# kleinzcy/speech_signal_processing

Hardware: AMD Instinct MI355X
Metric: MFCC frames/s (one fused pass: framing .. DCT + delta + delta-delta, 39-d) (higher is better)
Workload: dtype f32; 1 GPU; configs[1]: 100000 x 3 s synthetic 16 kHz utterances per GPU, 39-d MFCC (+delta+delta-delta), 400/160/512, 24 mel; utterances_per_gpu=100000, frames_per_gpu=29800000, d_out=39, parallelism=utterance-sharded x1, world_size_observed=1

## Files before the change

### speech_signal_processing_amd/csrc/mfcc.hpp

```cpp
#pragma once
#include "common.hpp"

namespace ssp {

struct MfccChunk {
    int32_t utt;
    int32_t t0;
    int32_t n;
    int32_t pad;
};

struct MfccArgs {
    const float* samples;
    const int64_t* sample_off;
    const int64_t* frame_off;
    float* out;
    float* lm_out;
    const MfccChunk* chunks;
    float* utt_max;
    const float* window;
    const float2* twiddle;
    const int32_t* filt_lo4;
    const float* filt_wT;
    const int32_t* filt_grp;
    int32_t filt_w4_total;
    int32_t dct_identity;
    int32_t dct_ncp;
    const float* dct;
    const float* dctT;
    int32_t win_len, hop, n_fft, n_filt, n_ceps, d_out;
    int32_t frame_mode, preemph_mode, spec_power, log_mode, floor_mode, delta_order, delta_N, cmvn;
    float preemph, spec_scale, eps, top_db, delta_inv_denom;
    int32_t lds_logmel_off, lds_ceps_off, lds_dlt_off, lds_ddl_off, lds_lmrows_off, lds_stats_off, lds_tw_off;
    int32_t lds_dct_off;
    int32_t lds_wt_off;
    int32_t lm_stride;
    int32_t n_chunks;
    int32_t prefetch;
};

constexpr int MFCC_FAST_MAX_PASS = 4;

struct FastArgs {
    const float2* tw16;
    const float2* wpost;
    const float* melw;
    const int32_t* mel_lo;
    const int32_t* mel_id;
    const float* dctT;
    int32_t mel_steps[MFCC_FAST_MAX_PASS];
    int32_t mel_blocks[MFCC_FAST_MAX_PASS];
    int32_t lm_pad;
    int32_t n_pass, q_pass, total_steps, n_filt4;
    float ddw[17];
    int32_t slen;
    int32_t stage_floats;
    int32_t ceps_rows;
    int32_t off_win, off_tw16, off_wpost, off_melw, off_mello, off_melid, off_dct, off_ceps, off_stats, off_wave, wave_bytes;
    float pscale;
    float one_minus_a;
    const float* pc_w;
    const int32_t* pc_ofs;
    const float* pc_mask;
    const int32_t* pc_fid;
    int32_t melv;
    int32_t mel_ns;
    float log_add, log_max, log_k;
    float* ceps_scratch;
    int32_t* work_counter;
    int32_t* redo_flags;
    int32_t ceps_stride;
    int32_t n_chunks;
};

struct StreamArgs {
    const float* dctA;
    int32_t* work_counter;
    int32_t* redo_flags;
    int32_t n_chunks;
    int32_t wave_bytes;
    int32_t stage_bytes;
    int32_t table_bytes;
    int32_t tstep;
    const float* dense_w;
};

int launch_mfcc_generic(const MfccArgs& args, int n_chunks, size_t lds_bytes, int n_waves, int num_cu, hipStream_t stream);
int launch_cmvn(const float* in, float* out, const int64_t* frame_off_dev, int64_t n_utt, int dim, int64_t max_T, hipStream_t stream);
int launch_topdb_dct(const float* logmel, const int64_t* frame_off_dev, int64_t n_utt, const MfccChunk* chunks, int n_chunks,
                     const float* utt_max, int n_filt, int n_ceps, const float* dct, float top_db, float* out, hipStream_t stream);
    

}

struct ssp_mfcc_plan {
    ssp_ctx* ctx = nullptr;
    ssp_mfcc_cfg cfg{};
    int32_t d_out = 0;
    bool reproducible = false;
    ssp::DevBuf window, twiddle, filt_lo4, filt_grp, filt_wT, dct, dctT, fbank_dense;
    int32_t max_filt_len = 0;
    uint64_t checked_sseg = 0, checked_fseg = 0;
    uint64_t cache_sseg = 0;
    uint64_t cache_fseg = 0;
    int cache_variant = -1;
    int cache_request = -1;
    bool cache_split_cmvn = false;
    bool cache_split_topdb = false;
    ssp::DevBuf lm_scratch, umax_scratch;
    int cache_chunk_frames = 0;
    size_t cache_lds = 0;
    int cache_waves = 4;
    int32_t cache_n_chunks = 0;
    std::vector<int32_t> cache_chunk_first;
    ssp::DevBuf chunks;
    ssp::MfccArgs args{};
    bool fast_ready = false;
    int64_t fast_max_samples = 0;
    ssp::FastArgs fast{};
    ssp::DevBuf f_tw16, f_wpost, f_melw, f_mello, f_melid, f_dct, f_pcw, f_pcofs, f_pcmask, f_pcfid, f_scratch, f_counter;
    bool stream_ready = false;
    ssp::DevBuf s_dctA, s_dense;
    bool cache_s2k_fused = false;
    bool s2k_ready = false;
    int32_t s2k_steps = 0, s2k_steps1 = 0;
    ssp::DevBuf s2k_twA, s2k_twB, s2k_twS, s2k_mel, s2k_minfo;
};

namespace ssp {
bool mfcc_fast_supported(const ssp_mfcc_cfg& cfg);
int build_fast_tables(ssp_mfcc_plan* plan);
size_t mfcc_fast_lds(const ssp_mfcc_cfg& cfg, FastArgs& f, int chunk_frames);
int mfcc_fast_max_chunk(const ssp_mfcc_cfg& cfg, const FastArgs& f);
int launch_mfcc_fast(const MfccArgs& args, ssp_mfcc_plan* plan, int n_chunks, int chunk_frames, hipStream_t stream);
bool mfcc_stream_supported(const ssp_mfcc_plan* plan);
bool mfcc_s2k_supported(const ssp_mfcc_plan* plan);
int build_s2k_tables(ssp_mfcc_plan* plan);
bool mfcc_s2k_fuses(const ssp_mfcc_plan* plan, int64_t max_T, int chunk_frames);
int launch_mfcc_s2k(const MfccArgs& args, ssp_mfcc_plan* plan, int n_chunks, hipStream_t stream);
bool mfcc_stream_dense(const ssp_mfcc_plan* plan);
bool mfcc_stream_fuses_cmvn(const ssp_mfcc_plan* plan);
int build_stream_tables(ssp_mfcc_plan* plan);
int launch_mfcc_stream(const MfccArgs& args, ssp_mfcc_plan* plan, int n_chunks, hipStream_t stream, bool dry_run = false);
}
```

### speech_signal_processing_amd/csrc/mfcc_plan.hip

```cpp
#include <chrono>
#include <cmath>
#include <cstdlib>

#include "mfcc.hpp"

namespace ssp {

static int validate_cfg(const ssp_mfcc_cfg* c) {
    if (!c) SSP_FAIL(SSP_ERR_INVALID, "mfcc: null cfg");
    if (c->n_fft < 64 || c->n_fft > 2048 || (c->n_fft & (c->n_fft - 1)))
        SSP_FAIL(SSP_ERR_UNSUPPORTED, "mfcc: n_fft=%d must be a power of two in [64, 2048]", c->n_fft);
    if (c->win_len < 1 || c->win_len > c->n_fft) SSP_FAIL(SSP_ERR_INVALID, "mfcc: win_len=%d not in [1, n_fft]", c->win_len);
    if (c->hop < 1) SSP_FAIL(SSP_ERR_INVALID, "mfcc: hop < 1");
    if (c->n_filt < 1 || c->n_filt > 512) SSP_FAIL(SSP_ERR_INVALID, "mfcc: n_filt=%d not in [1,512]", c->n_filt);
    if (c->n_ceps < 1 || c->n_ceps > 128) SSP_FAIL(SSP_ERR_INVALID, "mfcc: n_ceps=%d not in [1,128]", c->n_ceps);
    if (c->frame_mode < 0 || c->frame_mode > 2) SSP_FAIL(SSP_ERR_INVALID, "mfcc: frame_mode");
    if (c->frame_mode == 2 && c->win_len != c->n_fft)
        SSP_FAIL(SSP_ERR_UNSUPPORTED, "mfcc: centred framing needs win_len == n_fft");
    if (c->preemph_mode < 0 || c->preemph_mode > 1) SSP_FAIL(SSP_ERR_INVALID, "mfcc: preemph_mode");
    if (c->spec_power != 1 && c->spec_power != 2) SSP_FAIL(SSP_ERR_INVALID, "mfcc: spec_power must be 1 or 2");
    if (c->log_mode < 0 || c->log_mode > 2) SSP_FAIL(SSP_ERR_INVALID, "mfcc: log_mode");
    if (c->floor_mode < 0 || c->floor_mode > 2) SSP_FAIL(SSP_ERR_INVALID, "mfcc: floor_mode");
    if (c->delta_order < 0 || c->delta_order > 2) SSP_FAIL(SSP_ERR_INVALID, "mfcc: delta_order must be 0, 1 or 2");
    if (c->delta_order > 0 && (c->delta_N < 1 || c->delta_N > 8))
// ... 94 lines not shown
            MfccArgs probe = p->args;
            probe.cmvn = (c.cmvn != 0 && !split_cmvn) ? 1 : 0;
            const int prc = launch_mfcc_stream(probe, p, 0, nullptr, true);
            if (prc != SSP_OK) return prc;
        }
    } else if (variant == 2) {
        FastArgs tmp = p->fast;
        const int cap = mfcc_fast_max_chunk(c, tmp);
        ch = (int)std::min<int64_t>(std::max<int64_t>(max_T, 1), std::min(512, cap));
        if (whole) {
            ch = (int)std::max<int64_t>(max_T, 1);
            if (ch > cap) {
                split_cmvn = true;
                whole = false;
                ch = (int)std::min<int64_t>(std::max<int64_t>(max_T, 1), std::min(512, cap));
            }
        }
        lds = mfcc_fast_lds(c, tmp, ch);
        if (lds > lds_cap) SSP_FAIL(SSP_ERR_UNSUPPORTED, "mfcc(fast): LDS footprint %zu B exceeds 160 KiB", lds);
    } else {
        MfccArgs tmp = p->args;
        size_t half_cap = (size_t)(c.n_fft >= 2048 ? 80 : (c.n_fft >= 1024 ? 53 : 40)) * 1024;
        if (const char* e = getenv("SSP_GENERIC_LDS_CAP_KB")) half_cap = (size_t)atoi(e) * 1024;
        auto chunk_for = [&](const ssp_mfcc_cfg& cc) {
            int k = (int)std::min<int64_t>(std::max<int64_t>(max_T, 1), 512);
            while (k > 16 && generic_lds_layout(cc, k, 4, &tmp) > half_cap) k = (k * 3) / 4;
            return k;
        };
        nw = 4;
        ch = chunk_for(c);
        if (whole) {
            ch = (int)std::max<int64_t>(max_T, 1);
            if (generic_lds_layout(c, ch, 8, &tmp) <= lds_cap) {
                nw = 8;
            } else if (generic_lds_layout(c, ch, 4, &tmp) > lds_cap) {
                if (c.top_db >= 0.f) {
                    if (c.delta_order != 0 || c.cmvn)
                        SSP_FAIL(SSP_ERR_UNSUPPORTED,
                                 "mfcc: top_db with deltas / cmvn needs a whole utterance per workgroup; %lld frames exceed the 160 KiB LDS",
                                 (long long)max_T);
                    split_topdb = true;
                } else {
                    split_cmvn = true;
                }
                whole = false;
                ch = chunk_for(c);
                if (split_topdb) {
                    ssp_mfcc_cfg c2 = c;
                    c2.top_db = -1.f;
                    ch = chunk_for(c2);
                }
            }
        }
        {
            ssp_mfcc_cfg c2 = c;
            if (split_topdb) c2.top_db = -1.f;
            lds = generic_lds_layout(c2, ch, nw, &p->args);
        }
        if (lds > lds_cap) SSP_FAIL(SSP_ERR_UNSUPPORTED, "mfcc: LDS footprint %zu B exceeds 160 KiB", lds);
    }
    std::vector<MfccChunk> chunks;
    chunks.reserve((size_t)fseg->n);
    int64_t tail_from = fseg->n;
#ifndef SSP_NO_TAIL_SPLIT
    if (variant == 3 && !(c.cmvn != 0 && !split_cmvn) && !getenv("SSP_MFCC_NO_TAIL_SPLIT")) {
        const int64_t waves = (int64_t)p->ctx->num_cu * 12;
        if (fseg->n >= 4 * waves) tail_from = fseg->n - waves;
    }
#endif
    p->cache_chunk_first.assign((size_t)fseg->n + 1, 0);
    for (int64_t u = 0; u < fseg->n; ++u) {
        const int64_t T = fseg->host[u + 1] - fseg->host[u];
        if (T > INT32_MAX) SSP_FAIL(SSP_ERR_UNSUPPORTED, "mfcc: utterance %lld has too many frames", (long long)u);
        p->cache_chunk_first[(size_t)u] = (int32_t)std::min<size_t>(chunks.size(), (size_t)INT32_MAX);
        int64_t chu = ch;
        if (u >= tail_from && T >= 64) chu = std::min<int64_t>(ch, ((T + 1) / 2 + 15) / 16 * 16);
        const int pad = (variant == 3 && (!small_batch || repro)) ? 12 : 0;
        for (int64_t t0 = 0; t0 < T; t0 += chu)
            chunks.push_back(MfccChunk{(int32_t)u, (int32_t)t0, (int32_t)std::min<int64_t>(chu, T - t0), t0 > 0 ? pad : 0});
    }
    if (chunks.size() > (size_t)INT32_MAX) SSP_FAIL(SSP_ERR_UNSUPPORTED, "mfcc: too many chunks");
    p->cache_chunk_first[(size_t)fseg->n] = (int32_t)chunks.size();
    SSP_TRY(upload(p->chunks, chunks, p->ctx->stream));
    SSP_HIP(hipStreamSynchronize(p->ctx->stream));
    p->fast_max_samples = sseg->max_len();
    p->cache_n_chunks = (int32_t)chunks.size();
    p->cache_chunk_frames = ch;
    p->cache_lds = lds;
    p->cache_waves = nw;
    p->cache_sseg = sseg->serial;
    p->cache_fseg = fseg->serial;
    p->cache_variant = variant;
    p->cache_split_cmvn = split_cmvn;
    p->cache_split_topdb = split_topdb;
    return SSP_OK;
}

}

using namespace ssp;

extern "C" {

int ssp_mfcc_num_frames(const ssp_mfcc_cfg* cfg, int64_t n_samples, int64_t* n_frames) {
    if (!cfg || !n_frames || n_samples < 0) SSP_FAIL(SSP_ERR_INVALID, "ssp_mfcc_num_frames: bad argument");
    if (cfg->hop < 1 || cfg->frame_mode < 0 || cfg->frame_mode > 2) SSP_FAIL(SSP_ERR_INVALID, "ssp_mfcc_num_frames: bad cfg");
    *n_frames = frames_for(*cfg, n_samples);
    return SSP_OK;
}

int ssp_mfcc_out_dim(const ssp_mfcc_cfg* cfg, int32_t* d_out) {
    if (!cfg || !d_out) SSP_FAIL(SSP_ERR_INVALID, "ssp_mfcc_out_dim: null");
    *d_out = cfg->n_ceps * (1 + cfg->delta_order);
    return SSP_OK;
}

int ssp_mfcc_plan_create(ssp_ctx* ctx, const ssp_mfcc_cfg* cfg, const float* window, const float* fbank,
                         const float* dct, ssp_mfcc_plan** out) {
    ssp::TraceRange trace_("ssp_mfcc_plan_create");
    if (!out) SSP_FAIL(SSP_ERR_INVALID, "ssp_mfcc_plan_create: null out");
    *out = nullptr;
    SSP_TRY(use_ctx(ctx));
    SSP_TRY(validate_cfg(cfg));
    if (!window || !fbank || !dct) SSP_FAIL(SSP_ERR_INVALID, "ssp_mfcc_plan_create: null table");
    ssp_mfcc_plan* p = new (std::nothrow) ssp_mfcc_plan;
    if (!p) SSP_FAIL(SSP_ERR_NOMEM, "mfcc plan: host alloc");
    p->ctx = ctx;
    p->cfg = *cfg;
    p->d_out = cfg->n_ceps * (1 + cfg->delta_order);
    const int n_fft = cfg->n_fft, nb = n_fft / 2 + 1;

    std::vector<float> win(n_fft, 0.f);
    for (int i = 0; i < cfg->win_len; ++i) win[i] = window[i];
    std::vector<float2> tw(n_fft);
    for (int k = 0; k < n_fft; ++k) {
        const double ang = -2.0 * M_PI * (double)k / (double)n_fft;
        tw[k] = make_float2((float)cos(ang), (float)sin(ang));
    }
    std::vector<int32_t> lo(cfg->n_filt), len(cfg->n_filt), ofs(cfg->n_filt);
    std::vector<float> w;
    int32_t maxlen = 0;
    for (int j = 0; j < cfg->n_filt; ++j) {
        const float* row = fbank + (size_t)j * nb;
        int first = -1, last = -1;
        for (int k = 0; k < nb; ++k)
            if (row[k] != 0.f) {
                if (first < 0) first = k;
                last = k;
            }
        lo[j] = first < 0 ? 0 : first;
        len[j] = first < 0 ? 0 : last - first + 1;
        ofs[j] = (int32_t)w.size();
        for (int k = 0; k < len[j]; ++k) w.push_back(row[lo[j] + k]);
        maxlen = std::max(maxlen, len[j]);
    }
    p->max_filt_len = maxlen;
    const int n_grp = (cfg->n_filt + 63) / 64;
    std::vector<int32_t> lo4(cfg->n_filt);
    std::vector<float> wT;
    MfccArgs& ga = p->args;
    const int buf_floats = n_fft + n_fft / 16;
    std::vector<int32_t> grp(16, 0);
    for (int g = 0; g < n_grp; ++g) {
        const int j1 = std::min(cfg->n_filt, g * 64 + 64);
        int32_t steps = 2, taps = 0;
        for (int pass = 0; pass < 8; ++pass) {
// ... 493 lines not shown
```

### speech_signal_processing_amd/csrc/mfcc_stream_kernel.hpp

```cpp
#pragma once
#include <algorithm>
#include <cmath>
#include <cstdlib>
#include <type_traits>

#include "mfcc.hpp"
#include "cplx.hpp"

namespace ssp {

namespace {
typedef unsigned v2u __attribute__((ext_vector_type(2)));
typedef __attribute__((address_space(3))) const volatile v2f* lds_cv2f_t;
typedef __attribute__((address_space(3))) const volatile float* lds_cvf_t;
constexpr int ZROW = 128;
constexpr int ZFRAME = 16 * ZROW;
constexpr int LM_OFF = 1792;
constexpr int RING_FRAMES = 24;
constexpr int RING_ROW = 64;
constexpr int STREAM_WAVES = 4;
#ifndef SSP_S_PSHIFT
#define SSP_S_PSHIFT 64
#endif
constexpr int PSH = SSP_S_PSHIFT;
static_assert(4 * (256 + 24) + PSH <= LM_OFF - 192, "shifted P row: piece reads must stay below the log-mel rows");
#define SSP_STR_(x) #x
#define SSP_STR(x) SSP_STR_(x)

__device__ __forceinline__ float stream_log(const FastArgs& f, float v) {
    return __builtin_amdgcn_logf(fmaxf(v + f.log_add, f.log_max)) * f.log_k;
}

__device__ __forceinline__ float delta_weight(float t, float tp, float Tm1, float half_inv) {
    const float lo = tp <= 0.f ? -1.0e6f : tp;
    const float hi = tp >= Tm1 ? 1.0e6f : tp;
    const float a = fmaxf(lo, t - 2.f), b = fminf(hi, t + 2.f);
    const float cnt = fmaxf(b - a + 1.f, 0.f);
    const float w = cnt * (a + b - 2.f * t) * half_inv;
    return (tp < 0.f || tp > Tm1) ? 0.f : w;
}
}

template <int NZ, int POWER, int PRE, int MELV, int KS, int NS, int OCC, int CM, int WALK>
__global__ __launch_bounds__(64 * STREAM_WAVES, OCC) void mfcc_stream512_kernel(MfccArgs a, FastArgs f, StreamArgs sa) {
    extern __shared__ __attribute__((aligned(16))) char smem[];
    if (WALK && sa.work_counter[1] == 0) return;
    const int tid = threadIdx.x, lane = tid & 63;
    const int wave = __builtin_amdgcn_readfirstlane(tid >> 6);
    const int g = lane >> 4, j = lane & 15;
    constexpr int nc = 13;
    constexpr int mel_ns = NS;

    char* zbuf = smem + wave * sa.wave_bytes;
    float* stage = reinterpret_cast<float*>(zbuf + 4 * ZFRAME);
    char* ring = zbuf + 4 * ZFRAME + sa.stage_bytes;

    v2f wreg[NZ];
#pragma unroll
    for (int n1 = 0; n1 < NZ; ++n1) wreg[n1] = *reinterpret_cast<const v2f*>(a.window + 32 * n1 + 2 * j);
#pragma unroll
    for (int n1 = 0; n1 < NZ; ++n1) wreg[n1] = edge_row_taps(wreg[n1], 32 * n1 + 2 * j, a.win_len);
#ifndef SSP_STREAM_NTW
#define SSP_STREAM_NTW 15
#endif
#ifndef SSP_STREAM_NTW_CM
#define SSP_STREAM_NTW_CM 12
#endif
#ifndef SSP_STREAM_NWP
#define SSP_STREAM_NWP 8
#endif
    constexpr int NTW = OCC >= 3 ? (CM ? SSP_STREAM_NTW_CM : ((MELV <= 3 && NS <= 2) ? SSP_STREAM_NTW : ((MELV >= 4 && NS >= 4) ? 8 : 9))) : 15, NWP = OCC >= 3 ? SSP_STREAM_NWP : 8;
    static_assert(NTW >= 8, "rows above NTW take W^((k1 - 8) j) W^(8 j): W^(8 j) = twr[7] must be resident");
    v2f twr[NTW], wpr[NWP];
#pragma unroll
    for (int k1 = 1; k1 <= NTW; ++k1) twr[k1 - 1] = *reinterpret_cast<const v2f*>(&f.tw16[k1 * 16 + j]);
    float dA[KS];
#pragma unroll
    for (int s = 0; s < KS; ++s) dA[s] = sa.dctA[s * 64 + lane];
#pragma unroll
    for (int i = 0; i < NWP; ++i) wpr[i] = *reinterpret_cast<const v2f*>(&f.wpost[i * 16 + j]);
    constexpr bool DENSE = MELV == 0;
    constexpr int MV = DENSE ? 1 : MELV;
    v4f mw[MV];
    int mofs[MV];
    v2f mk01 = v2f{0.f, 0.f}, mk23 = v2f{0.f, 0.f};
    int mfid = -1;
    v4f dw[DENSE ? 6 : 1][4];
    float dw256[DENSE ? 6 : 1];
    if (DENSE) {
#pragma unroll
        for (int k = 0; k < 6; ++k) {
#pragma unroll
            for (int i = 0; i < 4; ++i) dw[DENSE ? k : 0][i] = *reinterpret_cast<const v4f*>(sa.dense_w + ((size_t)lane * 6 + k) * 20 + 4 * i);
            dw256[DENSE ? k : 0] = sa.dense_w[((size_t)lane * 6 + k) * 20 + 16];
        }
    } else {
#pragma unroll
        for (int i = 0; i < MV; ++i) {
            mw[i] = *reinterpret_cast<const v4f*>(f.pc_w + ((size_t)lane * MV + i) * 4);
            mofs[i] = f.pc_ofs[lane * MV + i];
        }
        mk01 = *reinterpret_cast<const v2f*>(f.pc_mask + lane * 4);
        mk23 = NS > 2 ? *reinterpret_cast<const v2f*>(f.pc_mask + lane * 4 + 2) : v2f{0.f, 0.f};
        mfid = f.pc_fid[lane];
    }

    const int hop = a.hop;
    const float pre = PRE ? a.preemph : 0.f;
    const float npre = -pre;
    const int n_piece = (f.slen + 255) >> 8;
    const bool has_half = (f.slen & 255) != 0 && (f.slen & 255) <= 128;
    const int n_full = has_half ? n_piece - 1 : n_piece;
    const int dord = a.delta_order;
    const int Dd = a.d_out;
    const float half_inv = 0.5f * a.delta_inv_denom;
    const uint32_t stage_lds = __builtin_amdgcn_readfirstlane((uint32_t)(uintptr_t)(lds_ptr_t)stage);

#ifdef SSP_S_CLOCK
    const unsigned long long ck0 = __builtin_amdgcn_s_memtime(), rt0 = __builtin_amdgcn_s_memrealtime();
#endif
    uint64_t wm = 0;
    int wblk = blockIdx.x * STREAM_WAVES + wave, wbase = 0;
    for (;;) {
        int cidx = 0;
        if constexpr (WALK) {
            bool done = false;
            while (wm == 0) {
                if ((int64_t)wblk * 64 >= sa.n_chunks) {
                    done = true;
                    break;
                }
                const int idx = wblk * 64 + lane;
                const int fl = idx < sa.n_chunks ? sa.redo_flags[idx] : 0;
                wm = __builtin_amdgcn_ballot_w64(fl != 0);
                wbase = wblk * 64;
                wblk += gridDim.x * STREAM_WAVES;
            }
            if (done) break;
            cidx = __builtin_amdgcn_readfirstlane(wbase + __builtin_ctzll(wm));
            wm &= wm - 1;
        } else {
            if (lane == 0) cidx = atomicAdd(sa.work_counter, 1);
            cidx = __builtin_amdgcn_readfirstlane(cidx);
            if (cidx >= sa.n_chunks) break;
        }
        const MfccChunk ch = a.chunks[cidx];
        const int64_t s0 = a.sample_off[ch.utt];
        const int64_t N = a.sample_off[ch.utt + 1] - s0;
        const int64_t f0 = a.frame_off[ch.utt];
        const int T = __builtin_amdgcn_readfirstlane((int)(a.frame_off[ch.utt + 1] - f0));
        const int t0 = __builtin_amdgcn_readfirstlane(ch.t0), n = __builtin_amdgcn_readfirstlane(ch.n);
        const int H = dord > 0 ? 4 : 0;
        const int Hlo = dord > 0 ? H + __builtin_amdgcn_readfirstlane(ch.pad) : 0;
        const int ta = max(t0 - Hlo, 0), tb = min(t0 + n + H, T);
        const int R = tb - ta;
        const int nquads = (R + 3) >> 2;
        const int E = t0 + n - ta;
        const int n_steps = (E + 4 + 15) >> 4;
        const int Q = DENSE ? nquads : 4 * n_steps;
        const float Tm1 = (float)(T - 1);

        const uint64_t xaddr = reinterpret_cast<uint64_t>(a.samples + s0);
        const uint32_t xlo = __builtin_amdgcn_readfirstlane((uint32_t)xaddr), xhi = __builtin_amdgcn_readfirstlane((uint32_t)(xaddr >> 32));
        const int xbytes = __builtin_amdgcn_readfirstlane((int)(N * 4));
        const __amdgpu_buffer_rsrc_t rs = __builtin_amdgcn_make_buffer_rsrc(
            reinterpret_cast<float*>(((uint64_t)xhi << 32) | xlo), 0, xbytes, 0x00020000);
        const uint64_t oaddr = reinterpret_cast<uint64_t>(a.out + (size_t)f0 * Dd);
        const uint32_t olo = __builtin_amdgcn_readfirstlane((uint32_t)oaddr), ohi = __builtin_amdgcn_readfirstlane((uint32_t)(oaddr >> 32));
        const __amdgpu_buffer_rsrc_t ro = __builtin_amdgcn_make_buffer_rsrc(
            reinterpret_cast<float*>(((uint64_t)ohi << 32) | olo), 0, __builtin_amdgcn_readfirstlane(T * Dd * 4), 0x00020000);

        auto prefetch = [&](int q) {
            const int vo = (ta + 4 * q) * hop * 4 + lane * 16;
            const lds_ptr_t lp = (lds_ptr_t)(uintptr_t)stage_lds;
            if (n_full > 0) __builtin_amdgcn_raw_ptr_buffer_load_lds(rs, lp, 16, vo, 0, 0, 0);
            if (n_full > 1) __builtin_amdgcn_raw_ptr_buffer_load_lds(rs, lp, 16, vo, 0, 1024, 0);
            if (n_full > 2) __builtin_amdgcn_raw_ptr_buffer_load_lds(rs, lp, 16, vo, 0, 2048, 0);
            if (n_full > 3) __builtin_amdgcn_raw_ptr_buffer_load_lds(rs, lp, 16, vo, 0, 3072, 0);
            if (n_full > 4) __builtin_amdgcn_raw_ptr_buffer_load_lds(rs, (lds_ptr_t)(uintptr_t)(stage_lds + 4096), 16, vo + 4096, 0, 0, 0);
            if (has_half && lane < 32)
                __builtin_amdgcn_raw_ptr_buffer_load_lds(rs, (lds_ptr_t)(uintptr_t)(stage_lds + n_full * 1024), 16, vo + n_full * 1024, 0, 0, 0);
        };

        {
            float zz = 0.f;
            asm volatile("" : "+v"(zz));
            v4f z4 = v4f{zz, zz, zz, zz};
            *reinterpret_cast<v4f*>(ring + lane * 16) = z4;
            if (lane < (RING_FRAMES * RING_ROW - 1024) / 16) *reinterpret_cast<v4f*>(ring + 1024 + lane * 16) = z4;
        }
        prefetch(0);
        int stores_pending = 0;
        int cm_nf = WALK;
        float cs1[CM ? 3 : 1] = {}, cs2[CM ? 3 : 1] = {};
        float piv = 0.f;

        typedef v2f zarr_t[16];
        typedef v2f pfarr_t[NZ];
        typedef float pmarr_t[PRE ? NZ : 1];
        constexpr int NH = (NZ + 1) / 2;
        auto wait_dma = [&]() {
#ifndef SSP_S_NOWAIT
            if (stores_pending == 0) asm volatile("s_waitcnt vmcnt(0)" ::: "memory");
            else if (stores_pending == 2) asm volatile("s_waitcnt vmcnt(2)" ::: "memory");
            else if (stores_pending == 4) asm volatile("s_waitcnt vmcnt(4)" ::: "memory");
            else if (stores_pending == 6) asm volatile("s_waitcnt vmcnt(6)" ::: "memory");
            else if (stores_pending == 9) asm volatile("s_waitcnt vmcnt(9)" ::: "memory");
            else asm volatile("s_waitcnt vmcnt(13)" ::: "memory");
#endif
            stores_pending = 0;
        };
        auto stage_read_a = [&](pfarr_t& pf, pmarr_t& pm) {
            const uint32_t sp = stage_lds + (g * hop + 2 * j) * 4;
#pragma unroll
            for (int n1 = 0; n1 < NH; ++n1) {
                pf[n1] = *(lds_cv2f_t)(uintptr_t)(sp + 128 * n1);
#ifdef SSP_S_PM64
                if (PRE) pm[n1] = (*(lds_cv2f_t)(uintptr_t)(sp + 128 * n1 - 8)).y;
#else
                if (PRE) pm[n1] = *(lds_cvf_t)(uintptr_t)(sp + 128 * n1 - 4);
#endif
            }
        };
        auto stage_read_b = [&](pfarr_t& pf, pmarr_t& pm) {
            const uint32_t sp = stage_lds + (g * hop + 2 * j) * 4;
#pragma unroll
            for (int n1 = NH; n1 < NZ; ++n1) {
                pf[n1] = *(lds_cv2f_t)(uintptr_t)(sp + 128 * n1);
#ifdef SSP_S_PM64
                if (PRE) pm[n1] = (*(lds_cv2f_t)(uintptr_t)(sp + 128 * n1 - 8)).y;
#else
                if (PRE) pm[n1] = *(lds_cvf_t)(uintptr_t)(sp + 128 * n1 - 4);
#endif
            }
        };
        auto win_rows = [&](zarr_t& z, pfarr_t& pf, pmarr_t& pm, auto lo_tag, auto hi_tag, auto edge_tag) {
            constexpr int LO = decltype(lo_tag)::value, HI = decltype(hi_tag)::value;
            constexpr int EDGE = decltype(edge_tag)::value;
#pragma unroll
            for (int n1 = LO; n1 < HI; ++n1) {
                if (n1 < NZ) {
                    v2f y = pf[n1 < NZ ? n1 : 0];
                    if (PRE) {
                        const float xm1 = pm[n1 < NZ ? n1 : 0], x0 = y.x, x1 = y.y;
                        y = v2f{__builtin_fmaf(npre, xm1, x0), __builtin_fmaf(npre, x0, x1)};
                    }
                    z[n1] = (EDGE == 1 || (EDGE == 2 && n1 == NZ - 1)) ? wmul_edge(y, wreg[n1 < NZ ? n1 : 0]) : y * wreg[n1 < NZ ? n1 : 0];
                } else {
                    z[n1] = v2f{0.f, 0.f};
                }
            }
        };
        auto window_a = [&](zarr_t& z, pfarr_t& pf, pmarr_t& pm, auto edge_tag) {
            if (PRE) pm[0] = (j == 0) ? pf[0].x : pm[0];
            win_rows(z, pf, pm, std::integral_constant<int, 0>{}, std::integral_constant<int, NH>{}, edge_tag);
        };
        auto window_b = [&](zarr_t& z, pfarr_t& pf, pmarr_t& pm, auto edge_tag) {
            win_rows(z, pf, pm, std::integral_constant<int, NH>{}, std::integral_constant<int, 16>{}, edge_tag);
        };
        auto fft_front = [&](zarr_t& z) {
            fft16_in<(NZ <= 13)>(z);
#pragma unroll
            for (int k1 = 1; k1 < 16; ++k1) {
                if (k1 <= NTW) {
                    z[k1] = cmul(z[k1], twr[(k1 - 1) % NTW]);
// ... 393 lines not shown
                    pfarr_t pf;
                    pmarr_t pm;
                    wait_dma();
                    stage_read_a(pf, pm);
                    asm volatile("s_waitcnt lgkmcnt(0)" ::: "memory");
                    window_a(z, pf, pm, std::integral_constant<int, 1>{});
                    stage_read_b(pf, pm);
                    asm volatile("s_waitcnt lgkmcnt(0)" ::: "memory");
                    prefetch(q + 1);
                    window_b(z, pf, pm, std::integral_constant<int, 1>{});
                    fft_front(z);
                    mel();
                    const v4f cq = dct_mfma();
                    ring_put(q, cq, true);
                } else {
                    ring_put(q, v4f{0.f, 0.f, 0.f, 0.f}, false);
                }
                if ((q & 3) == 3) time_step_nf(q >> 2);
            }
        } else {
#ifdef SSP_S_SEQ
            for (int q = 0; q < Q; ++q) {
                zarr_t z;
                pfarr_t pf;
                pmarr_t pm;
                if (q < nquads) {
                    wait_dma();
                    stage_read_a(pf, pm);
                    asm volatile("s_waitcnt lgkmcnt(0)" ::: "memory");
                    window_a(z, pf, pm, std::integral_constant<int, DENSE ? 2 : 0>{});
                    stage_read_b(pf, pm);
                    asm volatile("s_waitcnt lgkmcnt(0)" ::: "memory");
#ifndef SSP_S_NODMA
                    prefetch(q + 1);
#endif
                    window_b(z, pf, pm, std::integral_constant<int, DENSE ? 2 : 0>{});
                    fft_front(z);
                    mel();
                    const v4f cq = dct_mfma();
                    ring_put(q, cq, true);
                } else {
                    ring_put(q, v4f{0.f, 0.f, 0.f, 0.f}, false);
                }
#ifndef SSP_S_NOSTEP
                if ((q & 3) == 3) emit_step(q >> 2);
#endif
            }
#else
#ifdef SSP_S_PAD
            asm volatile(".rept " SSP_STR(SSP_S_PAD) "\n s_nop 0\n .endr");
#endif
            for (int q = 0; q < nquads; ++q) {
                zarr_t z;
                pfarr_t pf;
                pmarr_t pm;
                wait_dma();
                stage_read_a(pf, pm);
                const v4f cq = dct_mfma();
                asm volatile("s_waitcnt lgkmcnt(0)" ::: "memory");
                window_a(z, pf, pm, std::integral_constant<int, DENSE ? 2 : 0>{});
                stage_read_b(pf, pm);
                ring_put(q - 1, cq, q > 0);
                asm volatile("s_waitcnt lgkmcnt(0)" ::: "memory");
#ifndef SSP_S_NODMA
                prefetch(q + 1);
#endif
                window_b(z, pf, pm, std::integral_constant<int, DENSE ? 2 : 0>{});
                fft_front(z);
                mel();
#ifndef SSP_S_NOSTEP
                if ((q & 3) == 0 && q > 0) emit_step((q - 1) >> 2);
#endif
            }
            for (int qb = nquads - 1; qb < Q; ++qb) {
                v4f cq = v4f{0.f, 0.f, 0.f, 0.f};
                if (qb < nquads) cq = dct_mfma();
                ring_put(qb, cq, qb < nquads);
#ifndef SSP_S_NOSTEP
                if ((qb & 3) == 3) emit_step(qb >> 2);
#endif
            }
#endif
        }
        asm volatile("s_waitcnt vmcnt(0)" ::: "memory");
        if (CM) {
            int ol = lane;
            asm volatile("" : "+v"(ol));
            const int g = ol >> 4, j = ol & 15;
            float* ct = reinterpret_cast<float*>(ring);
            if (cm_nf) {
                double n1 = 0.0, a1 = 0.0, a2 = 0.0;
                const int col = ol < Dd ? ol : 0;
                for (int F0 = 0; F0 < T; F0 += 8) {
                    float v[8];
#pragma unroll
                    for (int k = 0; k < 8; ++k)
                        v[k] = __builtin_bit_cast(float, __builtin_amdgcn_raw_buffer_load_b32(ro, F0 + k < T ? ((F0 + k) * Dd + col) * 4 : 0x7ffffff0, 0, 1));
#pragma unroll
                    for (int k = 0; k < 8; ++k) {
                        const bool ok = F0 + k < T && v[k] == v[k];
                        const double d = ok ? (double)v[k] : 0.0;
                        n1 += ok ? 1.0 : 0.0;
                        a1 += d;
                        a2 += d * d;
                    }
                }
                const double mean = a1 / n1;
                const double var = a2 / n1 - mean * mean;
                double sd = __builtin_sqrt(var > 0.0 ? var : (var == var ? 0.0 : var));
                if (sd < 10.0 * 1.1920929e-07) sd = 1.0;
                if (ol < Dd) {
                    ct[ol] = (float)mean;
                    ct[48 + ol] = (float)(1.0 / sd);
                }
            } else
#pragma unroll
            for (int blk = 0; blk < 3; ++blk) {
                if (blk > dord) break;
                double a1 = (double)cs1[CM ? blk : 0], a2 = (double)cs2[CM ? blk : 0];
                auto xor_add = [&](double v, int m) -> double {
                    const v2u b = __builtin_bit_cast(v2u, v);
                    const int addr = (ol ^ m) << 2;
                    const v2u o = v2u{(unsigned)__builtin_amdgcn_ds_bpermute(addr, (int)b.x), (unsigned)__builtin_amdgcn_ds_bpermute(addr, (int)b.y)};
                    return v + __builtin_bit_cast(double, o);
                };
                a1 = xor_add(a1, 16);
                a2 = xor_add(a2, 16);
                a1 = xor_add(a1, 32);
                a2 = xor_add(a2, 32);
                const double m0 = a1 / (double)T;
                const double mean = m0 + (blk == 0 ? (double)piv : 0.0);
                const double var = a2 / (double)T - m0 * m0;
                double sd = __builtin_sqrt(var > 0.0 ? var : (var == var ? 0.0 : var));
                if (sd < 10.0 * 1.1920929e-07) sd = 1.0;
                if (g == 0 && j < nc) {
                    ct[blk * nc + j] = (float)mean;
                    ct[48 + blk * nc + j] = (float)(1.0 / sd);
                }
            }
            asm volatile("s_waitcnt lgkmcnt(0)" ::: "memory");
            const int tot = T * Dd;
            auto rewrite = [&](auto wtag) {
                constexpr int W = decltype(wtag)::value, B = 16;
                const int n_el = tot / W;
                const int step = (64 * W) % Dd;
                int c = (ol * W) % Dd;
                for (int i0 = 0; i0 < n_el; i0 += 64 * B) {
                    v2f v[B];
#pragma unroll
                    for (int k = 0; k < B; ++k) {
                        const int idx = i0 + 64 * k + ol;
                        const int off = idx < n_el ? idx * (4 * W) : 0x7ffffff0;
                        if (W == 2) v[k] = __builtin_bit_cast(v2f, __builtin_amdgcn_raw_buffer_load_b64(ro, off, 0, 1));
                        else v[k] = v2f{__builtin_bit_cast(float, __builtin_amdgcn_raw_buffer_load_b32(ro, off, 0, 1)), 0.f};
                    }
#pragma unroll
                    for (int k = 0; k < B; ++k) {
                        const int idx = i0 + 64 * k + ol;
                        const int off = idx < n_el ? idx * (4 * W) : 0x7ffffff0;
                        const int c1 = c + 1 == Dd ? 0 : c + 1;
                        const float m0 = ct[c], is0 = ct[48 + c];
                        if (W == 2) {
                            const float m1 = ct[c1], is1 = ct[48 + c1];
                            const v2f o = v2f{(v[k].x - m0) * is0, (v[k].y - m1) * is1};
                            __builtin_amdgcn_raw_buffer_store_b64(__builtin_bit_cast(v2u, o), ro, off, 0, 0);
                        } else {
                            __builtin_amdgcn_raw_buffer_store_b32(__builtin_bit_cast(unsigned, (v[k].x - m0) * is0), ro, off, 0, 0);
                        }
                        c += step;
                        c = c >= Dd ? c - Dd : c;
                    }
                }
            };
            if ((Dd & 1) == 0) rewrite(std::integral_constant<int, 2>{});
            else rewrite(std::integral_constant<int, 1>{});
            asm volatile("s_waitcnt vmcnt(0) lgkmcnt(0)" ::: "memory");
        }
    }
#ifdef SSP_S_CLOCK
    if (tid == 0) {
        const unsigned long long ck1 = __builtin_amdgcn_s_memtime(), rt1 = __builtin_amdgcn_s_memrealtime();
        atomicAdd(reinterpret_cast<unsigned long long*>(sa.work_counter + 8), ck1 - ck0);
        atomicAdd(reinterpret_cast<unsigned long long*>(sa.work_counter + 10), rt1 - rt0);
    }
#endif
}

static inline int stream_ks(const ssp_mfcc_cfg& c) { return (c.n_filt + 3) / 4 <= 6 ? 6 : 10; }

template <int WALK>
int launch_mfcc_stream_impl(const MfccArgs& args, ssp_mfcc_plan* p, int n_chunks, hipStream_t stream, bool dry_run) {
    if (n_chunks <= 0 && !dry_run) return SSP_OK;
    FastArgs f = p->fast;
    const ssp_mfcc_cfg& c = p->cfg;
    StreamArgs sa{};
    const int KS = stream_ks(c);
    f.lm_pad = 4 * KS - c.n_filt;
    if (f.lm_pad > 16 && f.melv != 0) SSP_FAIL(SSP_ERR_UNSUPPORTED, "mfcc(stream): %d filters leave more than 16 padded slots", c.n_filt);
    sa.dctA = p->s_dctA.as<float>();
    sa.dense_w = p->s_dense.as<float>();
    const int n_piece = (f.slen + 255) >> 8;
    const bool has_half = (f.slen & 255) != 0 && (f.slen & 255) <= 128;
    sa.stage_bytes = has_half ? (n_piece - 1) * 1024 + 512 : n_piece * 1024;
    sa.wave_bytes = 4 * ZFRAME + sa.stage_bytes + RING_FRAMES * RING_ROW;
    sa.table_bytes = 0;
    sa.n_chunks = n_chunks;
    if (!dry_run) {
        SSP_TRY(p->f_counter.reserve(64 + (size_t)std::max(n_chunks, 1) * sizeof(int32_t)));
        sa.work_counter = p->f_counter.as<int32_t>();
        sa.redo_flags = sa.work_counter + 16;
    }
    size_t lds = (size_t)sa.table_bytes + (size_t)STREAM_WAVES * sa.wave_bytes;
    if (const char* e = getenv("SSP_MFCC_LDS_PAD")) lds = std::min<size_t>(160 * 1024, lds + (size_t)atoi(e));
    if (lds > 160 * 1024) SSP_FAIL(SSP_ERR_UNSUPPORTED, "mfcc(stream): LDS footprint %zu B exceeds 160 KiB", lds);
    if ((int64_t)p->fast_max_samples * 4 > INT32_MAX) SSP_FAIL(SSP_ERR_UNSUPPORTED, "mfcc(stream): utterance too long for 32-bit offsets");
    const int nz = c.win_len <= 416 ? 13 : 16, pw = c.spec_power, pr = c.preemph_mode ? 1 : 0;
    const int cm = args.cmvn != 0 ? 1 : 0;
    const int occ = (nz == 13 && KS == 6 && lds <= 53248 && f.melv != 0 && (!cm || (f.melv <= 3 && f.mel_ns <= 2))) ? 3 : 2;
    const int wg_waves = STREAM_WAVES;
    bool launched = false;
#define SSP_STREAM_CASE(NZ_, PW_, PR_, MV_, KS_, OCC_) SSP_STREAM_CASE_CM(NZ_, PW_, PR_, MV_, KS_, OCC_, 0)
#define SSP_STREAM_CASE_CM(NZ_, PW_, PR_, MV_, KS_, OCC_, CM_)                                                        \
    if (!launched && dry_run && nz == NZ_ && pw == PW_ && pr == PR_ && f.melv == MV_ && KS == KS_ && occ == OCC_ && cm == CM_) \
        launched = true;                                                                                                \
    if (!launched && nz == NZ_ && pw == PW_ && pr == PR_ && f.melv == MV_ && KS == KS_ && occ == OCC_ && cm == CM_) {   \
        auto* kfn = f.mel_ns <= 2 ? mfcc_stream512_kernel<NZ_, PW_, PR_, MV_, KS_, 2, OCC_, CM_, WALK>                    \
                                  : mfcc_stream512_kernel<NZ_, PW_, PR_, MV_, KS_, 4, OCC_, CM_, WALK>;                   \
        if (lds > 64 * 1024)                                                                                            \
            SSP_HIP(hipFuncSetAttribute(reinterpret_cast<const void*>(kfn), hipFuncAttributeMaxDynamicSharedMemorySize, (int)lds)); \
        int per_cu = 0;                                                                                                 \
        SSP_HIP(hipOccupancyMaxActiveBlocksPerMultiprocessor(&per_cu, kfn, 64 * wg_waves, lds));                        \
        const int grid = std::min((n_chunks + wg_waves - 1) / wg_waves, std::max(1, per_cu) * p->ctx->num_cu);          \
        if (!WALK) SSP_HIP(hipMemsetAsync(sa.work_counter, 0, 64 + (size_t)n_chunks * 4, stream));     \
        if (getenv("SSP_DEBUG")) fprintf(stderr, "[ssp] mfcc stream%s: grid %d (%d per CU), lds %zu\n", WALK ? " (second kernel)" : "", grid, per_cu, lds); \
        hipLaunchKernelGGL(kfn, dim3(grid), dim3(64 * wg_waves), lds, stream, args, f, sa);                             \
        launched = true;                                                                                                \
    }
#define SSP_STREAM_CASE_CM3(MV_)                                                                                          \
    if (!launched && dry_run && nz == 13 && pw == 2 && pr == 1 && f.melv == MV_ && KS == 6 && occ == 3 && cm == 1) launched = true; \
    if (!launched && nz == 13 && pw == 2 && pr == 1 && f.melv == MV_ && KS == 6 && occ == 3 && cm == 1) {                   \
        auto* kfn = mfcc_stream512_kernel<13, 2, 1, MV_, 6, 2, 3, 1, WALK>;                                               \
        int per_cu = 0;                                                                                                   \
        SSP_HIP(hipOccupancyMaxActiveBlocksPerMultiprocessor(&per_cu, kfn, 64 * wg_waves, lds));                          \
        const int grid = std::min((n_chunks + wg_waves - 1) / wg_waves, std::max(1, per_cu) * p->ctx->num_cu);            \
        if (!WALK) SSP_HIP(hipMemsetAsync(sa.work_counter, 0, 64 + (size_t)n_chunks * 4, stream));                            \
        hipLaunchKernelGGL(kfn, dim3(grid), dim3(64 * wg_waves), lds, stream, args, f, sa);                               \
        launched = true;                                                                                                  \
    }
    SSP_STREAM_CASE_CM3(2) SSP_STREAM_CASE_CM3(3)
#undef SSP_STREAM_CASE_CM3
    SSP_STREAM_CASE_CM(13, 2, 1, 2, 6, 2, 1) SSP_STREAM_CASE_CM(13, 2, 1, 3, 6, 2, 1) SSP_STREAM_CASE_CM(13, 2, 1, 4, 6, 2, 1)
    if constexpr (!WALK) {
        SSP_STREAM_CASE(13, 2, 1, 0, 6, 2)
    }
#ifdef SSP_FAST_MINIMAL
    SSP_STREAM_CASE(13, 2, 1, 3, 6, 3)
    SSP_STREAM_CASE(16, 1, 0, 3, 10, 2)
    SSP_STREAM_CASE(16, 1, 0, 5, 10, 2)
#else
#define SSP_STREAM_MV(NZ_, PW_, PR_, KS_, OCC_)                                                                         \
    SSP_STREAM_CASE(NZ_, PW_, PR_, 2, KS_, OCC_) SSP_STREAM_CASE(NZ_, PW_, PR_, 3, KS_, OCC_) SSP_STREAM_CASE(NZ_, PW_, PR_, 4, KS_, OCC_)
    SSP_STREAM_MV(13, 2, 1, 6, 3)
    SSP_STREAM_MV(13, 2, 0, 6, 3)
    SSP_STREAM_MV(13, 1, 0, 6, 3)
    SSP_STREAM_MV(16, 2, 1, 6, 2)
    SSP_STREAM_MV(16, 2, 0, 6, 2)
    SSP_STREAM_MV(16, 1, 0, 6, 2)
    SSP_STREAM_MV(16, 2, 1, 10, 2)
    SSP_STREAM_MV(16, 2, 0, 10, 2)
    SSP_STREAM_MV(16, 1, 0, 10, 2)
    SSP_STREAM_MV(13, 2, 1, 10, 2)
    SSP_STREAM_CASE(16, 2, 1, 5, 10, 2) SSP_STREAM_CASE(16, 2, 0, 5, 10, 2) SSP_STREAM_CASE(16, 1, 0, 5, 10, 2)
    SSP_STREAM_CASE(13, 2, 1, 5, 10, 2)
#undef SSP_STREAM_MV
#endif
#undef SSP_STREAM_CASE
#undef SSP_STREAM_CASE_CM
    if (!launched) SSP_FAIL(SSP_ERR_UNSUPPORTED, "mfcc(stream): no kernel instance for this cfg");
    if (dry_run) return SSP_OK;
    SSP_HIP(hipGetLastError());
    return SSP_OK;
}

}
```

Before: 3.024 billion frames/s.

## Prefetch next chunk descriptor and claim work one chunk ahead in stream kernel

Precomputes a packed 48-byte per-chunk descriptor on the host so the stream kernel reads everything it needs with three scalar 16-byte loads. The MfccChunk, sample_off and frame_off chains are no longer read per chunk. Each wave now claims its next chunk via a buffer atomic one iteration ahead and loads that chunk's descriptor before the vmcnt wait, hiding atomic and descriptor latency behind the current chunk's work. Look-ahead stops near the tail (ahead_until) to keep load balance. The cost is extra plan memory and a tighter coupling between launch chunks and the plan's table.

```diff
diff --git a/speech_signal_processing_amd/csrc/mfcc.hpp b/speech_signal_processing_amd/csrc/mfcc.hpp
--- a/speech_signal_processing_amd/csrc/mfcc.hpp
+++ b/speech_signal_processing_amd/csrc/mfcc.hpp
@@ -9,6 +9,18 @@
     int32_t n;
     int32_t pad;
 };
+
+struct alignas(16) StreamChunk {
+    int64_t s0;
+    int32_t xbytes;
+    int32_t ta;
+    int64_t f0;
+    int32_t T;
+    int32_t t0;
+    int32_t n;
+    int32_t rsv[3];
+};
+static_assert(sizeof(StreamChunk) == 48, "three 16-byte scalar loads");
 
 struct MfccArgs {
     const float* samples;
@@ -83,6 +95,8 @@
     int32_t table_bytes;
     int32_t tstep;
     const float* dense_w;
+    const StreamChunk* desc;
+    int32_t ahead_until;
 };
 
 int launch_mfcc_generic(const MfccArgs& args, int n_chunks, size_t lds_bytes, int n_waves, int num_cu, hipStream_t stream);
@@ -114,6 +128,7 @@
     int32_t cache_n_chunks = 0;
     std::vector<int32_t> cache_chunk_first;
     ssp::DevBuf chunks;
+    ssp::DevBuf stream_chunks;
     ssp::MfccArgs args{};
     bool fast_ready = false;
     int64_t fast_max_samples = 0;
diff --git a/speech_signal_processing_amd/csrc/mfcc_plan.hip b/speech_signal_processing_amd/csrc/mfcc_plan.hip
--- a/speech_signal_processing_amd/csrc/mfcc_plan.hip
+++ b/speech_signal_processing_amd/csrc/mfcc_plan.hip
@@ -200,6 +200,23 @@
     if (chunks.size() > (size_t)INT32_MAX) SSP_FAIL(SSP_ERR_UNSUPPORTED, "mfcc: too many chunks");
     p->cache_chunk_first[(size_t)fseg->n] = (int32_t)chunks.size();
     SSP_TRY(upload(p->chunks, chunks, p->ctx->stream));
+    std::vector<StreamChunk> recs;
+    if (variant == 3) {
+        recs.resize(chunks.size());
+        for (size_t i = 0; i < chunks.size(); ++i) {
+            const MfccChunk& k = chunks[i];
+            StreamChunk& r = recs[i];
+            r = StreamChunk{};
+            r.s0 = sseg->host[(size_t)k.utt];
+            r.xbytes = (int32_t)std::min<int64_t>((sseg->host[(size_t)k.utt + 1] - r.s0) * 4, INT32_MAX);
+            r.ta = c.delta_order > 0 ? std::max(k.t0 - 4 - k.pad, 0) : k.t0;
+            r.f0 = fseg->host[(size_t)k.utt];
+            r.T = (int32_t)(fseg->host[(size_t)k.utt + 1] - r.f0);
+            r.t0 = k.t0;
+            r.n = k.n;
+        }
+        SSP_TRY(upload(p->stream_chunks, recs, p->ctx->stream));
+    }
     SSP_HIP(hipStreamSynchronize(p->ctx->stream));
     p->fast_max_samples = sseg->max_len();
     p->cache_n_chunks = (int32_t)chunks.size();
diff --git a/speech_signal_processing_amd/csrc/mfcc_stream_kernel.hpp b/speech_signal_processing_amd/csrc/mfcc_stream_kernel.hpp
--- a/speech_signal_processing_amd/csrc/mfcc_stream_kernel.hpp
+++ b/speech_signal_processing_amd/csrc/mfcc_stream_kernel.hpp
@@ -13,6 +13,8 @@
 typedef unsigned v2u __attribute__((ext_vector_type(2)));
 typedef __attribute__((address_space(3))) const volatile v2f* lds_cv2f_t;
 typedef __attribute__((address_space(3))) const volatile float* lds_cvf_t;
+typedef int v4i __attribute__((ext_vector_type(4)));
+typedef __attribute__((address_space(4))) const v4i* const_v4i_t;
 constexpr int ZROW = 128;
 constexpr int ZFRAME = 16 * ZROW;
 constexpr int LM_OFF = 1792;
@@ -121,8 +123,27 @@
 #endif
     uint64_t wm = 0;
     int wblk = blockIdx.x * STREAM_WAVES + wave, wbase = 0;
+    int c_cur = -1, c_nx = -1;
+    v4i cw0 = v4i{0, 0, 0, 0};
+    v4i cw1 = v4i{0, 0, 0, 0};
+    int cwn = 0;
+    auto in_table = [&](int c) -> bool { return c >= 0 && c < sa.n_chunks; };
+    const const_v4i_t desc = (const_v4i_t)(uintptr_t)sa.desc;
+    auto sample_addr = [&](v4i w) -> uint64_t {
+        return reinterpret_cast<uint64_t>(a.samples) + ((((uint64_t)(uint32_t)w.y << 32) | (uint32_t)w.x) << 2);
+    };
+    const __amdgpu_buffer_rsrc_t rcnt = __builtin_amdgcn_make_buffer_rsrc(sa.work_counter, 0, 4, 0x00020000);
+    auto claim = [&](bool on) -> int {
+        int ol = lane;
+        asm volatile("" : "+v"(ol));
+        return __builtin_amdgcn_raw_ptr_buffer_atomic_add_i32(1, rcnt, (on && ol == 0) ? 0 : 0x7ffffff0, 0, 0);
+    };
     for (;;) {
         int cidx = 0;
+        int64_t f0;
+        int T, t0, n, ta;
+        uint32_t xlo, xhi;
+        int xbytes;
         if constexpr (WALK) {
             bool done = false;
             while (wm == 0) {
@@ -139,20 +160,34 @@
             if (done) break;
             cidx = __builtin_amdgcn_readfirstlane(wbase + __builtin_ctzll(wm));
             wm &= wm - 1;
+            const MfccChunk ch = a.chunks[cidx];
+            const int64_t s0 = a.sample_off[ch.utt];
+            const int64_t N = a.sample_off[ch.utt + 1] - s0;
+            f0 = a.frame_off[ch.utt];
+            T = __builtin_amdgcn_readfirstlane((int)(a.frame_off[ch.utt + 1] - f0));
+            t0 = __builtin_amdgcn_readfirstlane(ch.t0), n = __builtin_amdgcn_readfirstlane(ch.n);
+            ta = max(t0 - (dord > 0 ? 4 + __builtin_amdgcn_readfirstlane(ch.pad) : 0), 0);
+            const uint64_t xaddr = reinterpret_cast<uint64_t>(a.samples + s0);
+            xlo = __builtin_amdgcn_readfirstlane((uint32_t)xaddr), xhi = __builtin_amdgcn_readfirstlane((uint32_t)(xaddr >> 32));
+            xbytes = __builtin_amdgcn_readfirstlane((int)(N * 4));
         } else {
-            if (lane == 0) cidx = atomicAdd(sa.work_counter, 1);
-            cidx = __builtin_amdgcn_readfirstlane(cidx);
-            if (cidx >= sa.n_chunks) break;
+            if (c_cur < 0) {
+                c_cur = __builtin_amdgcn_readfirstlane(claim(true));
+                if (c_cur >= sa.n_chunks) break;
+                cw0 = desc[3 * c_cur];
+                cw1 = desc[3 * c_cur + 1];
+                cwn = desc[3 * c_cur + 2].x;
+                c_nx = c_cur < sa.ahead_until ? __builtin_amdgcn_readfirstlane(claim(true)) : -1;
+            }
+            cidx = c_cur;
+            const uint64_t xaddr = sample_addr(cw0);
+            xlo = (uint32_t)xaddr, xhi = (uint32_t)(xaddr >> 32), xbytes = cw0.z, ta = cw0.w;
+            f0 = (int64_t)(((uint64_t)(uint32_t)cw1.y << 32) | (uint32_t)cw1.x);
+            T = cw1.z, t0 = cw1.w, n = cwn;
         }
-        const MfccChunk ch = a.chunks[cidx];
-        const int64_t s0 = a.sample_off[ch.utt];
-        const int64_t N = a.sample_off[ch.utt + 1] - s0;
-        const int64_t f0 = a.frame_off[ch.utt];
-        const int T = __builtin_amdgcn_readfirstlane((int)(a.frame_off[ch.utt + 1] - f0));
-        const int t0 = __builtin_amdgcn_readfirstlane(ch.t0), n = __builtin_amdgcn_readfirstlane(ch.n);
+        const bool have_nx = !WALK && in_table(c_nx);
         const int H = dord > 0 ? 4 : 0;
-        const int Hlo = dord > 0 ? H + __builtin_amdgcn_readfirstlane(ch.pad) : 0;
-        const int ta = max(t0 - Hlo, 0), tb = min(t0 + n + H, T);
+        const int tb = min(t0 + n + H, T);
         const int R = tb - ta;
         const int nquads = (R + 3) >> 2;
         const int E = t0 + n - ta;
@@ -160,9 +195,6 @@
         const int Q = DENSE ? nquads : 4 * n_steps;
         const float Tm1 = (float)(T - 1);
 
-        const uint64_t xaddr = reinterpret_cast<uint64_t>(a.samples + s0);
-        const uint32_t xlo = __builtin_amdgcn_readfirstlane((uint32_t)xaddr), xhi = __builtin_amdgcn_readfirstlane((uint32_t)(xaddr >> 32));
-        const int xbytes = __builtin_amdgcn_readfirstlane((int)(N * 4));
         const __amdgpu_buffer_rsrc_t rs = __builtin_amdgcn_make_buffer_rsrc(
             reinterpret_cast<float*>(((uint64_t)xhi << 32) | xlo), 0, xbytes, 0x00020000);
         const uint64_t oaddr = reinterpret_cast<uint64_t>(a.out + (size_t)f0 * Dd);
@@ -170,17 +202,18 @@
         const __amdgpu_buffer_rsrc_t ro = __builtin_amdgcn_make_buffer_rsrc(
             reinterpret_cast<float*>(((uint64_t)ohi << 32) | olo), 0, __builtin_amdgcn_readfirstlane(T * Dd * 4), 0x00020000);
 
-        auto prefetch = [&](int q) {
-            const int vo = (ta + 4 * q) * hop * 4 + lane * 16;
+        auto prefetch_at = [&](const __amdgpu_buffer_rsrc_t rx, int sb) {
+            const int vo = sb + lane * 16;
             const lds_ptr_t lp = (lds_ptr_t)(uintptr_t)stage_lds;
-            if (n_full > 0) __builtin_amdgcn_raw_ptr_buffer_load_lds(rs, lp, 16, vo, 0, 0, 0);
-            if (n_full > 1) __builtin_amdgcn_raw_ptr_buffer_load_lds(rs, lp, 16, vo, 0, 1024, 0);
-            if (n_full > 2) __builtin_amdgcn_raw_ptr_buffer_load_lds(rs, lp, 16, vo, 0, 2048, 0);
-            if (n_full > 3) __builtin_amdgcn_raw_ptr_buffer_load_lds(rs, lp, 16, vo, 0, 3072, 0);
-            if (n_full > 4) __builtin_amdgcn_raw_ptr_buffer_load_lds(rs, (lds_ptr_t)(uintptr_t)(stage_lds + 4096), 16, vo + 4096, 0, 0, 0);
+            if (n_full > 0) __builtin_amdgcn_raw_ptr_buffer_load_lds(rx, lp, 16, vo, 0, 0, 0);
+            if (n_full > 1) __builtin_amdgcn_raw_ptr_buffer_load_lds(rx, lp, 16, vo, 0, 1024, 0);
+            if (n_full > 2) __builtin_amdgcn_raw_ptr_buffer_load_lds(rx, lp, 16, vo, 0, 2048, 0);
+            if (n_full > 3) __builtin_amdgcn_raw_ptr_buffer_load_lds(rx, lp, 16, vo, 0, 3072, 0);
+            if (n_full > 4) __builtin_amdgcn_raw_ptr_buffer_load_lds(rx, (lds_ptr_t)(uintptr_t)(stage_lds + 4096), 16, vo + 4096, 0, 0, 0);
             if (has_half && lane < 32)
-                __builtin_amdgcn_raw_ptr_buffer_load_lds(rs, (lds_ptr_t)(uintptr_t)(stage_lds + n_full * 1024), 16, vo + n_full * 1024, 0, 0, 0);
-        };
+                __builtin_amdgcn_raw_ptr_buffer_load_lds(rx, (lds_ptr_t)(uintptr_t)(stage_lds + n_full * 1024), 16, vo + n_full * 1024, 0, 0, 0);
+        };
+        auto prefetch = [&](int q) { prefetch_at(rs, (ta + 4 * q) * hop * 4); };
 
         {
             float zz = 0.f;
@@ -740,7 +773,19 @@
             }
 #endif
         }
+        v4i bw0 = v4i{0, 0, 0, 0}, bw1 = v4i{0, 0, 0, 0};
+        int bwn = 0, c_new = -1;
+        const bool do_claim = have_nx && c_nx < sa.ahead_until;
+        if constexpr (!WALK) {
+            if (have_nx) {
+                bw0 = desc[3 * c_nx];
+                bw1 = desc[3 * c_nx + 1];
+                bwn = desc[3 * c_nx + 2].x;
+            }
+            c_new = claim(do_claim);
+        }
         asm volatile("s_waitcnt vmcnt(0)" ::: "memory");
+        if constexpr (!WALK) c_new = do_claim ? __builtin_amdgcn_readfirstlane(c_new) : (c_nx >= sa.n_chunks ? c_nx : -1);
         if (CM) {
             int ol = lane;
             asm volatile("" : "+v"(ol));
@@ -834,6 +879,14 @@
             else rewrite(std::integral_constant<int, 1>{});
             asm volatile("s_waitcnt vmcnt(0) lgkmcnt(0)" ::: "memory");
         }
+        if constexpr (!WALK) {
+            if (c_nx >= sa.n_chunks) break;
+            c_cur = have_nx ? c_nx : -1;
+            cw0 = bw0;
+            cw1 = bw1;
+            cwn = bwn;
+            c_nx = c_new;
+        }
     }
 #ifdef SSP_S_CLOCK
     if (tid == 0) {
@@ -845,6 +898,9 @@
 }
 
 static inline int stream_ks(const ssp_mfcc_cfg& c) { return (c.n_filt + 3) / 4 <= 6 ? 6 : 10; }
+static inline int stream_ahead_until(int n_chunks, int waves, int cut) {
+    return (int64_t)n_chunks >= 4 * (int64_t)waves ? (int)std::max<int64_t>(0, n_chunks - (int64_t)cut * waves) : n_chunks;
+}
 
 template <int WALK>
 int launch_mfcc_stream_impl(const MfccArgs& args, ssp_mfcc_plan* p, int n_chunks, hipStream_t stream, bool dry_run) {
@@ -863,6 +919,13 @@
     sa.wave_bytes = 4 * ZFRAME + sa.stage_bytes + RING_FRAMES * RING_ROW;
     sa.table_bytes = 0;
     sa.n_chunks = n_chunks;
+    if (!dry_run && !WALK) {
+        if ((int64_t)n_chunks * 3 > INT32_MAX) SSP_FAIL(SSP_ERR_UNSUPPORTED, "mfcc(stream): too many chunks");
+        const ptrdiff_t c0 = args.chunks - p->chunks.as<MfccChunk>();
+        if (c0 < 0 || (size_t)(c0 + n_chunks) * sizeof(StreamChunk) > p->stream_chunks.bytes)
+            SSP_FAIL(SSP_ERR_INVALID, "mfcc(stream): the launch's chunks are not the plan's work table");
+        sa.desc = p->stream_chunks.as<StreamChunk>() + c0;
+    }
     if (!dry_run) {
         SSP_TRY(p->f_counter.reserve(64 + (size_t)std::max(n_chunks, 1) * sizeof(int32_t)));
         sa.work_counter = p->f_counter.as<int32_t>();
@@ -870,6 +933,10 @@
     }
     size_t lds = (size_t)sa.table_bytes + (size_t)STREAM_WAVES * sa.wave_bytes;
     if (const char* e = getenv("SSP_MFCC_LDS_PAD")) lds = std::min<size_t>(160 * 1024, lds + (size_t)atoi(e));
+    int grid_cap = INT32_MAX;
+    if (const char* e = getenv("SSP_MFCC_STREAM_GRID")) grid_cap = std::max(1, atoi(e));
+    int ahead_cut = 2;
+    if (const char* e = getenv("SSP_MFCC_STREAM_AHEAD_CUT")) ahead_cut = std::max(0, atoi(e));
     if (lds > 160 * 1024) SSP_FAIL(SSP_ERR_UNSUPPORTED, "mfcc(stream): LDS footprint %zu B exceeds 160 KiB", lds);
     if ((int64_t)p->fast_max_samples * 4 > INT32_MAX) SSP_FAIL(SSP_ERR_UNSUPPORTED, "mfcc(stream): utterance too long for 32-bit offsets");
     const int nz = c.win_len <= 416 ? 13 : 16, pw = c.spec_power, pr = c.preemph_mode ? 1 : 0;
@@ -888,7 +955,8 @@
             SSP_HIP(hipFuncSetAttribute(reinterpret_cast<const void*>(kfn), hipFuncAttributeMaxDynamicSharedMemorySize, (int)lds)); \
         int per_cu = 0;                                                                                                 \
         SSP_HIP(hipOccupancyMaxActiveBlocksPerMultiprocessor(&per_cu, kfn, 64 * wg_waves, lds));                        \
-        const int grid = std::min((n_chunks + wg_waves - 1) / wg_waves, std::max(1, per_cu) * p->ctx->num_cu);          \
+        const int grid = std::min(grid_cap, std::min((n_chunks + wg_waves - 1) / wg_waves, std::max(1, per_cu) * p->ctx->num_cu)); \
+        sa.ahead_until = stream_ahead_until(n_chunks, std::max(1, per_cu) * p->ctx->num_cu * wg_waves, ahead_cut);              \
         if (!WALK) SSP_HIP(hipMemsetAsync(sa.work_counter, 0, 64 + (size_t)n_chunks * 4, stream));     \
         if (getenv("SSP_DEBUG")) fprintf(stderr, "[ssp] mfcc stream%s: grid %d (%d per CU), lds %zu\n", WALK ? " (second kernel)" : "", grid, per_cu, lds); \
         hipLaunchKernelGGL(kfn, dim3(grid), dim3(64 * wg_waves), lds, stream, args, f, sa);                             \
@@ -900,7 +968,8 @@
         auto* kfn = mfcc_stream512_kernel<13, 2, 1, MV_, 6, 2, 3, 1, WALK>;                                               \
         int per_cu = 0;                                                                                                   \
         SSP_HIP(hipOccupancyMaxActiveBlocksPerMultiprocessor(&per_cu, kfn, 64 * wg_waves, lds));                          \
-        const int grid = std::min((n_chunks + wg_waves - 1) / wg_waves, std::max(1, per_cu) * p->ctx->num_cu);            \
+        const int grid = std::min(grid_cap, std::min((n_chunks + wg_waves - 1) / wg_waves, std::max(1, per_cu) * p->ctx->num_cu)); \
+        sa.ahead_until = stream_ahead_until(n_chunks, std::max(1, per_cu) * p->ctx->num_cu * wg_waves, ahead_cut);                \
         if (!WALK) SSP_HIP(hipMemsetAsync(sa.work_counter, 0, 64 + (size_t)n_chunks * 4, stream));                            \
         hipLaunchKernelGGL(kfn, dim3(grid), dim3(64 * wg_waves), lds, stream, args, f, sa);                               \
         launched = true;                                                                                                  \
```

Measured after the change: 2.989 billion frames/s. 0.988x the previous value.
